# david-wb/tiny-diffusion

Measured on AMD Instinct MI355X. Metric: train images/s (q_sample+fwd+MSE+bwd+allreduce+Adam), MNIST 28x28 UNet fp32; 1000-step sample latency in `sample`, higher is better.
Workload: dtype f32; 1 GPU; diffusion.py unconditional MNIST 28x28 UNet, fp32, train step, batch 256/GPU (BASELINE.json configs[1]); global_batch=256, per_gpu_batch=256, parallelism=dp1

## Files before the change

### include/tdx.h

```cpp
#ifndef TDX_H
#define TDX_H

#include <stddef.h>
#include <stdint.h>

#ifdef __cplusplus
extern "C" {
#endif

#define TDX_VERSION 400

#define TDX_E_BADARG (-1)
#define TDX_E_SHAPE (-2)
#define TDX_E_WORKSPACE (-3)
#define TDX_E_STATE (-4)

typedef void* tdx_stream_t;

int tdx_version(void);
const char* tdx_error_string(int code);


int tdx_q_sample(const float* x0, const float* noise, const int64_t* t,
                 const float* sqrt_ac, const float* sqrt_1mac, float* x_t,
// ... 290 lines not shown
size_t tdx_vae_loss_scratch_bytes(void);
int tdx_vae_bce_logits_grad(const float* logits, const float* x, float* loss_out, float* d_logits, float* recon,
                            float gscale, int64_t n, void* scratch, tdx_stream_t stream);
int tdx_vae_kld_reparam_bwd(const float* mu, const float* logvar, const float* eps, const float* g_z, float* kld_out,
                            float* g_mu, float* g_logvar, float kld_weight, int64_t n, void* scratch,
                            tdx_stream_t stream);
int tdx_vae_reparameterize_philox(const float* mu, const float* logvar, float* z, float* eps_out, int64_t n,
                                  uint64_t seed, uint64_t offset, tdx_stream_t stream);
size_t tdx_vae_train_workspace_floats(int batch, int input_dim, int hidden_dim, int latent_dim);
int tdx_vae_loss_grads(const float* x, const void* const* params, void* const* grads, const float* eps, uint64_t seed,
                       uint64_t offset, float kld_weight, float gscale, float* out3, float* workspace, int batch,
                       int input_dim, int hidden_dim, int latent_dim, tdx_stream_t stream);

int tdx_layernorm_fwd(const float* x, const float* gamma, const float* beta, float* out,
                      float* mean, float* rstd, int M, int N, float eps, tdx_stream_t stream);
int tdx_layernorm_bwd(const float* gy, const float* x, const float* gamma, const float* mean,
                      const float* rstd, float* gx, float* dgamma, float* dbeta, int M, int N,
                      tdx_stream_t stream);
int tdx_act_fwd(const float* x, float* out, int64_t n, int kind, tdx_stream_t stream);
int tdx_act_bwd(const float* gy, const float* x, float* gx, int64_t n, int kind, tdx_stream_t stream);
int tdx_dropout(const float* x, float* out, int64_t n, int group, float p, uint64_t seed,
                uint64_t offset, tdx_stream_t stream);
int tdx_add(const float* a, const float* b, float* out, int64_t n, int64_t b_period, tdx_stream_t stream);
int tdx_embedding_fwd(const float* weight, const int64_t* idx, float* out, int M, int N,
                      tdx_stream_t stream);
int tdx_embedding_bwd(const float* g, const int64_t* idx, float* dweight, int M, int N, int num,
                      tdx_stream_t stream);

typedef struct tdx_transformer_shape {
  int batch, latent_dim, dim, num_heads, num_layers, num_classes;
  float dropout_p, ln_eps;
} tdx_transformer_shape;
size_t tdx_transformer_train_workspace_floats(const tdx_transformer_shape* shape);
int tdx_transformer_loss_grads(const tdx_transformer_shape* shape, const void* const* params, void* const* grads,
                               const float* z_t, const int64_t* t, const int64_t* y, const float* target,
                               const float* w_table, int train, uint64_t seed, uint64_t offset,
                               const uint64_t* rng_dev, float gscale, float* loss_out, float* eps_hat_out,
                               float* workspace, tdx_stream_t stream);

typedef struct tdx_unet tdx_unet;

int tdx_unet_create(tdx_unet** out, int max_batch, int num_classes);
enum { TDX_UNET_MNIST = 0, TDX_UNET_LAION = 1, TDX_UNET_LATENT_MLP = 2 };
int tdx_unet_create_ex(tdx_unet** out, int max_batch, int kind, int num_classes);
int tdx_unet_create_hw(tdx_unet** out, int max_batch, int kind, int num_classes, int hw);
int tdx_unet_create_full(tdx_unet** out, int max_batch, int kind, int num_classes, int hw, int time_dim);
typedef int (*tdx_allreduce_fn)(void* user, double* device_buffer, int n, tdx_stream_t stream);
int tdx_unet_set_bn_sync(tdx_unet* u, tdx_allreduce_fn fn, void* user, double* buffer);

int tdx_unet_set_streams(tdx_unet* u, int mode);

#define TDX_PREC_F32 0
#define TDX_PREC_BF16 1
int tdx_unet_set_precision(tdx_unet* u, int precision);
int tdx_unet_destroy(tdx_unet* u);
size_t tdx_unet_workspace_bytes(const tdx_unet* u, int batch, int mode);

int tdx_unet_forward(tdx_unet* u, const void* const* params, void* const* buffers,
                     const float* x, const int64_t* t, const void* cond, float* out,
                     void* workspace, size_t workspace_bytes, int batch, int mode,
                     tdx_stream_t stream);

int tdx_unet_backward_stages(void);
int tdx_unet_backward(tdx_unet* u, const void* const* params, void* const* grads,
                      const float* d_out, void* workspace, size_t workspace_bytes,
                      int batch, int stage_lo, int stage_hi, tdx_stream_t stream);
int tdx_unet_backward_join(tdx_unet* u, tdx_stream_t stream);
int tdx_unet_backward_mark(tdx_unet* u, int slot);
int tdx_unet_backward_wait_mark(tdx_unet* u, int slot, tdx_stream_t stream);
int tdx_unet_backward_sync_mark(tdx_unet* u, int slot);

int tdx_unet_request_input_grad(tdx_unet* u, float* g_x);

int tdx_timestep_embedding(const int64_t* t, float* out, int B, int dim, tdx_stream_t stream);
int tdx_timestep_embedding_f32(const float* t, float* out, int B, int dim, tdx_stream_t stream);

int tdx_time_mlp_fwd(const int64_t* t, const int64_t* y, const void* const* params, float* pre,
                     float* emb, float* t1, float* t2, float* t3, int batch, tdx_stream_t stream);
int tdx_time_mlp_bwd(const int64_t* t, const int64_t* y, const void* const* params,
                     void* const* grads, const float* pre, const float* emb, const float* g_t1,
                     const float* g_t2, const float* g_t3, float* scratch, int batch,
                     int num_classes, tdx_stream_t stream);

int tdx_unet_eval_step(tdx_unet* u, const void* const* params, void* const* buffers, float* x,
                       const void* cond, const float* z, const float* coef, int64_t* counter,
                       int32_t* t_idx, int64_t* t_vec, float* eps, int64_t n_elems,
                       void* workspace, size_t workspace_bytes, int batch, uint64_t philox_seed,
                       tdx_stream_t stream);

int tdx_unet_prepare_sampling(tdx_unet* u, const void* const* params, const void* cond, int batch, int T,
                              tdx_stream_t stream);

int tdx_unet_drop_sampling_tables(tdx_unet* u);

int tdx_unet_prepare_sampling_sched(tdx_unet* u, const void* const* params, const void* cond, int batch,
                                    const int64_t* tau, int S, tdx_stream_t stream);
int tdx_unet_eval_step_update(tdx_unet* u, const void* const* params, void* const* buffers, float* x,
                              const void* cond, const float* z, const float* coef, const int64_t* tau, int S,
                              int64_t* counter, int32_t* t_idx, int64_t* t_vec, float* eps, int64_t n_elems,
                              void* workspace, size_t workspace_bytes, int batch, uint64_t philox_seed, int form,
                              int guided, float w, float lo, float hi, float* hist, const float* known,
                              const float* mask, tdx_stream_t stream);
int tdx_unet_eval_step_update_dyn(tdx_unet* u, const void* const* params, void* const* buffers, float* x,
                                  const void* cond, const float* z, const float* coef, const int64_t* tau, int S,
                                  int64_t* counter, int32_t* t_idx, int64_t* t_vec, float* eps, int64_t n_elems,
                                  void* workspace, size_t workspace_bytes, int batch, uint64_t philox_seed, int form,
                                  int guided, float w, float lo, float hi, float* hist, const float* known,
                                  const float* mask, int rank, float frac, float* thr, tdx_stream_t stream);

int tdx_unet_tensor(const tdx_unet* u, int batch, const char* name, size_t* offset_floats,
                    size_t* numel);

int tdx_unet_pack(tdx_unet* u, const void* const* params, void* const* buffers,
                  tdx_stream_t stream);

int tdx_tune_set(const char* key, int value);
int tdx_tune_get(const char* key, int* value);
const char* tdx_tune_name(int index);

int tdx_diag_set_buffer(void* device_buffer, size_t bytes);
int tdx_diag_conv_occupancy(int tile);

int tdx_probe_mfma_f32(float* out, int iters, int blocks, tdx_stream_t stream);
int tdx_probe_stream_copy(const float* src, float* dst, int64_t n, tdx_stream_t stream);

#ifdef __cplusplus
}
#endif
#endif
```

### tiny_diffusion_amd/_lib.py

```python
from __future__ import annotations

import contextlib
import ctypes as C
import os

import torch

from . import _build

_c_float_p = C.c_void_p
_c_i64_p = C.c_void_p
_ptr = C.c_void_p


class TdxError(RuntimeError):
    pass


def _load():
    path = _build.LIB
    if not os.path.exists(path):
        if os.environ.get("TDX_NO_AUTOBUILD"):
            raise TdxError(
                f"{path} not found: build it with `python -m tiny_diffusion_amd._build` "
# ... 122 lines not shown
    "tdx_vae_decode": (C.c_int, [_ptr, _ptr, _ptr, _ptr, C.c_int, C.c_int, C.c_int, C.c_int, _ptr]),
    "tdx_vae_loss_scratch_bytes": (C.c_size_t, []),
    "tdx_vae_bce_logits_grad": (C.c_int, [_ptr] * 5 + [C.c_float, C.c_int64, _ptr, _ptr]),
    "tdx_vae_kld_reparam_bwd": (C.c_int, [_ptr] * 7 + [C.c_float, C.c_int64, _ptr, _ptr]),
    "tdx_vae_reparameterize_philox": (C.c_int, [_ptr] * 4 + [C.c_int64, C.c_uint64, C.c_uint64, _ptr]),
    "tdx_vae_train_workspace_floats": (C.c_size_t, [C.c_int] * 4),
    "tdx_vae_loss_grads": (C.c_int, [_ptr] * 4 + [C.c_uint64, C.c_uint64, C.c_float, C.c_float, _ptr, _ptr]
                           + [C.c_int] * 4 + [_ptr]),
    "tdx_layernorm_fwd": (C.c_int, [_ptr, _ptr, _ptr, _ptr, _ptr, _ptr, C.c_int, C.c_int, C.c_float, _ptr]),
    "tdx_layernorm_bwd": (C.c_int, [_ptr, _ptr, _ptr, _ptr, _ptr, _ptr, _ptr, _ptr, C.c_int, C.c_int, _ptr]),
    "tdx_act_fwd": (C.c_int, [_ptr, _ptr, C.c_int64, C.c_int, _ptr]),
    "tdx_act_bwd": (C.c_int, [_ptr, _ptr, _ptr, C.c_int64, C.c_int, _ptr]),
    "tdx_dropout": (C.c_int, [_ptr, _ptr, C.c_int64, C.c_int, C.c_float, C.c_uint64, C.c_uint64, _ptr]),
    "tdx_add": (C.c_int, [_ptr, _ptr, _ptr, C.c_int64, C.c_int64, _ptr]),
    "tdx_embedding_fwd": (C.c_int, [_ptr, _ptr, _ptr, C.c_int, C.c_int, _ptr]),
    "tdx_embedding_bwd": (C.c_int, [_ptr, _ptr, _ptr, C.c_int, C.c_int, C.c_int, _ptr]),
    "tdx_transformer_train_workspace_floats": (C.c_size_t, [_ptr]),
    "tdx_transformer_loss_grads": (C.c_int, [_ptr] * 8 + [C.c_int, C.c_uint64, C.c_uint64, _ptr, C.c_float] + [_ptr] * 4),
    "tdx_unet_create": (C.c_int, [C.POINTER(_ptr), C.c_int, C.c_int]),
    "tdx_unet_create_ex": (C.c_int, [C.POINTER(_ptr), C.c_int, C.c_int, C.c_int]),
    "tdx_unet_create_hw": (C.c_int, [C.POINTER(_ptr), C.c_int, C.c_int, C.c_int, C.c_int]),
    "tdx_unet_create_full": (C.c_int, [C.POINTER(_ptr), C.c_int, C.c_int, C.c_int, C.c_int, C.c_int]),
    "tdx_unet_set_bn_sync": (C.c_int, [_ptr, _ptr, _ptr, _ptr]),
    "tdx_unet_set_streams": (C.c_int, [_ptr, C.c_int]),
    "tdx_unet_set_precision": (C.c_int, [_ptr, C.c_int]),
    "tdx_pack_conv3x3_bf16": (C.c_int, [_ptr, _ptr, _ptr, C.c_int, C.c_int, _ptr]),
    "tdx_conv3x3_bf16_stat_tile_rows": (C.c_int, []),
    "tdx_conv3x3_fwd_bf16": (C.c_int, [_ptr, _ptr, _ptr, _ptr, C.c_int, C.c_int, C.c_int, C.c_int, C.c_int,
                                       C.c_int, _ptr, _ptr, _ptr, _ptr, _ptr, _ptr]),
    "tdx_conv3x3_wgrad_bf16": (C.c_int, [_ptr, _ptr, _ptr, C.c_int, C.c_int, C.c_int, C.c_int, C.c_int,
                                         C.c_int, _ptr, _ptr, _ptr]),
    "tdx_unet_destroy": (C.c_int, [_ptr]),
    "tdx_unet_workspace_bytes": (C.c_size_t, [_ptr, C.c_int, C.c_int]),
    "tdx_unet_forward": (C.c_int, [_ptr, _ptr, _ptr, _ptr, _ptr, _ptr, _ptr, _ptr, C.c_size_t, C.c_int,
                                   C.c_int, _ptr]),
    "tdx_unet_backward_stages": (C.c_int, []),
    "tdx_unet_backward": (C.c_int, [_ptr, _ptr, _ptr, _ptr, _ptr, C.c_size_t, C.c_int, C.c_int, C.c_int,
                                    _ptr]),
    "tdx_unet_backward_join": (C.c_int, [_ptr, _ptr]),
    "tdx_unet_backward_mark": (C.c_int, [_ptr, C.c_int]),
    "tdx_unet_backward_wait_mark": (C.c_int, [_ptr, C.c_int, _ptr]),
    "tdx_unet_backward_sync_mark": (C.c_int, [_ptr, C.c_int]),
    "tdx_unet_request_input_grad": (C.c_int, [_ptr, _ptr]),
    "tdx_unet_prepare_sampling": (C.c_int, [_ptr, _ptr, _ptr, C.c_int, C.c_int, _ptr]),
    "tdx_unet_drop_sampling_tables": (C.c_int, [_ptr]),
    "tdx_unet_prepare_sampling_sched": (C.c_int, [_ptr, _ptr, _ptr, C.c_int, _ptr, C.c_int, _ptr]),
    "tdx_initial_conv_input_grad": (C.c_int, [_ptr, _ptr, _ptr] + [C.c_int] * 5 + [_ptr]),
    "tdx_unet_eval_step": (C.c_int, [_ptr, _ptr, _ptr, _ptr, _ptr, _ptr, _ptr, _ptr, _ptr, _ptr, _ptr, C.c_int64,
                                     _ptr, C.c_size_t, C.c_int, C.c_uint64, _ptr]),
    "tdx_unet_eval_step_update": (C.c_int, [_ptr] * 8 + [C.c_int, _ptr, _ptr, _ptr, _ptr, C.c_int64, _ptr, C.c_size_t,
                                            C.c_int, C.c_uint64, C.c_int, C.c_int] + [C.c_float] * 3 + [_ptr] * 4),
    "tdx_p_sample_update": (C.c_int, [_ptr, _ptr, _ptr, C.c_int64, C.c_int, _ptr, _ptr, _ptr, _ptr, C.c_int, C.c_uint64,
                                      C.c_int, C.c_float, C.c_float, C.c_float, _ptr, _ptr, _ptr, _ptr, _ptr]),
    "tdx_x0_dyn_threshold": (C.c_int, [_ptr, _ptr, C.c_int, C.c_int, _ptr, _ptr, C.c_int, C.c_float, C.c_float, C.c_float,
                                       C.c_int, C.c_float, _ptr, _ptr]),
    "tdx_p_sample_update_dyn": (C.c_int, [_ptr, _ptr, _ptr, C.c_int64, C.c_int, _ptr, _ptr, _ptr, _ptr, C.c_int,
                                          C.c_uint64, C.c_int, C.c_float, C.c_float, C.c_float, _ptr, _ptr, _ptr, _ptr,
                                          _ptr, C.c_int, _ptr]),
    "tdx_unet_eval_step_update_dyn": (C.c_int, [_ptr] * 8 + [C.c_int, _ptr, _ptr, _ptr, _ptr, C.c_int64, _ptr, C.c_size_t,
                                                C.c_int, C.c_uint64, C.c_int, C.c_int] + [C.c_float] * 3 + [_ptr] * 3
                                      + [C.c_int, C.c_float, _ptr, _ptr]),
    "tdx_vlb_terms": (C.c_int, [_ptr] * 6 + [C.c_int, C.c_int] + [C.c_float] * 4 + [C.c_int, _ptr, C.c_int64, _ptr]),
    "tdx_p_sample_step_guided": (C.c_int, [_ptr, _ptr, _ptr, _ptr, _ptr, _ptr, C.c_int64, C.c_float, C.c_int,
                                           C.c_uint64, _ptr, _ptr]),
    "tdx_p_sample_step_x0": (C.c_int, [_ptr] * 7 + [C.c_int64, C.c_float, C.c_float, C.c_int, C.c_uint64, _ptr, _ptr]),
    "tdx_p_sample_step_x0_guided": (C.c_int, [_ptr] * 6 + [C.c_int64, C.c_float, C.c_float, C.c_float, C.c_int,
                                                           C.c_uint64, _ptr, _ptr]),
    "tdx_p_sample_step_ms": (C.c_int, [_ptr] * 6 + [C.c_int64, C.c_float, C.c_float, _ptr, _ptr]),
    "tdx_p_sample_step_ms_guided": (C.c_int, [_ptr] * 5 + [C.c_int64, C.c_float, C.c_float, C.c_float, _ptr, _ptr]),
    "tdx_p_sample_step_x0_masked": (C.c_int, [_ptr] * 9 + [C.c_int64, C.c_float, C.c_float, C.c_int, C.c_uint64, _ptr,
                                                           _ptr]),
    "tdx_p_sample_step_x0_guided_masked": (C.c_int, [_ptr] * 8 + [C.c_int64, C.c_float, C.c_float, C.c_float, C.c_int,
                                                                  C.c_uint64, _ptr, _ptr]),
    "tdx_p_sample_step_ms_masked": (C.c_int, [_ptr] * 8 + [C.c_int64, C.c_float, C.c_float, _ptr, _ptr]),
    "tdx_p_sample_step_ms_guided_masked": (C.c_int, [_ptr] * 7 + [C.c_int64, C.c_float, C.c_float, C.c_float, _ptr,
                                                                  _ptr]),
    "tdx_cond_drop_labels": (C.c_int, [_ptr, _ptr, C.c_int, C.c_float, C.c_uint64, C.c_uint64, _ptr]),
    "tdx_cond_drop_rows": (C.c_int, [_ptr, _ptr, C.c_int, C.c_int, C.c_float, C.c_uint64, C.c_uint64, _ptr]),
    "tdx_timestep_embedding": (C.c_int, [_ptr, _ptr, C.c_int, C.c_int, _ptr]),
    "tdx_timestep_embedding_f32": (C.c_int, [_ptr, _ptr, C.c_int, C.c_int, _ptr]),
    "tdx_time_mlp_fwd": (C.c_int, [_ptr, _ptr, _ptr, _ptr, _ptr, _ptr, _ptr, _ptr, C.c_int, _ptr]),
    "tdx_time_mlp_bwd": (C.c_int, [_ptr, _ptr, _ptr, _ptr, _ptr, _ptr, _ptr, _ptr, _ptr, _ptr, C.c_int, C.c_int,
                                   _ptr]),
    "tdx_conv3x3_dgrad": (C.c_int, [_ptr, _ptr, _ptr, C.c_int, C.c_int, C.c_int, C.c_int, C.c_int, _ptr]),
    "tdx_bn_apply_relu_fwd": (C.c_int, [_ptr, _ptr, C.c_int64, C.c_int, _ptr, _ptr, _ptr]),
    "tdx_unet_pack": (C.c_int, [_ptr, _ptr, _ptr, _ptr]),
    "tdx_unet_tensor": (C.c_int, [_ptr, C.c_int, C.c_char_p, C.POINTER(C.c_size_t), C.POINTER(C.c_size_t)]),
    "tdx_tune_set": (C.c_int, [C.c_char_p, C.c_int]),
    "tdx_tune_get": (C.c_int, [C.c_char_p, C.POINTER(C.c_int)]),
    "tdx_tune_name": (C.c_char_p, [C.c_int]),
    "tdx_diag_set_buffer": (C.c_int, [_ptr, C.c_size_t]),
    "tdx_probe_mfma_f32": (C.c_int, [_ptr, C.c_int, C.c_int, _ptr]),
    "tdx_probe_stream_copy": (C.c_int, [_ptr, _ptr, C.c_int64, _ptr]),
}

EXPORTS = tuple(_SIGS)
STEP_EPS, STEP_X0, STEP_MS = 0, 1, 2


def _bind():
    missing = []
    for name, (res, args) in _SIGS.items():
        try:
            fn = getattr(lib, name)
        except AttributeError:
            missing.append(name)
            continue
        fn.restype = res
        fn.argtypes = args
    if missing:
        raise TdxError(f"libtdx.so lacks symbols declared in include/tdx.h: {missing}")


_bind()


def _apply_env_tuning():
    spec = os.environ.get("TDX_TUNE", "")
    for item in filter(None, (x.strip() for x in spec.split(","))):
        key, _, val = item.partition("=")
        if lib.tdx_tune_set(key.encode(), int(val)) != 0:
            raise TdxError(f"unknown TDX_TUNE knob {key!r}")


_apply_env_tuning()


def check(code: int, what: str = "tdx"):
    if code != 0:
        msg = lib.tdx_error_string(code)
        raise TdxError(f"{what} failed: {msg.decode() if msg else code} ({code})")


def tune_get(key: str) -> int:
    value = C.c_int()
    if lib.tdx_tune_get(key.encode(), C.byref(value)) != 0:
        raise TdxError(f"unknown tuning knob {key!r}")
    return value.value


@contextlib.contextmanager
def tuned(**knobs):
    old = [(key, tune_get(key)) for key in knobs]
    try:
        for key, value in knobs.items():
            check(lib.tdx_tune_set(key.encode(), int(value)), f"tdx_tune_set({key})")
        yield
    finally:
        for key, value in reversed(old):
            check(lib.tdx_tune_set(key.encode(), value), f"tdx_tune_set({key})")


def ptr(t):
    return None if t is None else t.data_ptr()


def stream_ptr(device=None):
    return torch.cuda.current_stream(device).cuda_stream
```

### tiny_diffusion_amd/csrc/time_embed.hip

```cpp
#include "internal.h"

#define TD 256
#define TDL 768

__device__ static inline float silu_f(float x) { return x / (1.0f + expf(-x)); }
__device__ static inline float silu_grad_f(float x) {
  const float s = 1.0f / (1.0f + expf(-x));
  return s * (1.0f + x * (1.0f - s));
}

__device__ static inline void wave_dot4(const float* __restrict__ w0, int row_stride, const float4 v,
                                        int lane, float (&out)[4]) {
  float4 a[4];
#pragma unroll
  for (int k = 0; k < 4; ++k) a[k] = *reinterpret_cast<const float4*>(w0 + (size_t)k * row_stride + lane * 4);
#pragma unroll
  for (int k = 0; k < 4; ++k) out[k] = wave_sum(a[k].x * v.x + a[k].y * v.y + a[k].z * v.z + a[k].w * v.w);
}

__global__ void __launch_bounds__(256)
time_emb_kernel(const int64_t* __restrict__ t, const int64_t* __restrict__ y,
                const float* __restrict__ w1, const float* __restrict__ b1,
                const float* __restrict__ w2, const float* __restrict__ b2,
                const float* __restrict__ cls, float* __restrict__ pre_out,
// ... 162 lines not shown
    default: return TDX_E_SHAPE;
  }
  TDX_CHECK_LAUNCH();
  return 0;
}

static int time_embed_fwd_laion(const int64_t* t, const float* cond, const float* const* P, float* sin,
                                float* pre, float* emb, float* t1, float* t2, float* t3, int B, int td,
                                hipStream_t st) {
  sinusoid_kernel<int64_t><<<cdiv((int64_t)B * td, 256), 256, 0, st>>>(t, sin, B, td);
  TDX_CHECK_LAUNCH();
  int rc = linear_rows<false>(sin, P[TDX_P_TE0_W], P[TDX_P_TE0_B], nullptr, pre, B, td, td, st);
  if (rc) return rc;
  rc = linear_rows<true>(pre, P[TDX_P_TE2_W], P[TDX_P_TE2_B], cond, emb, B, td, td, st);
  if (rc) return rc;
  float* dst[3] = {t1, t2, t3};
  const int width[3] = {64, 128, 256};
  const int pw[3] = {TDX_P_TP1_W, TDX_P_TP2_W, TDX_P_TP3_W};
  for (int k = 0; k < 3; ++k) {
    rc = linear_rows<false>(emb, P[pw[k]], P[pw[k] + 1], nullptr, dst[k], B, width[k], td, st);
    if (rc) return rc;
  }
  return 0;
}

__global__ void time_l1_fwd_kernel(const int64_t* __restrict__ t, const float* __restrict__ w1,
                                   const float* __restrict__ b1, float* __restrict__ pre, float* __restrict__ tf,
                                   int B, int td) {
  const int i = blockIdx.x * blockDim.x + threadIdx.x;
  if (i >= B * td) return;
  const int n = i / td, j = i - n * td;
  const float v = (float)t[n];
  pre[i] = fmaf(w1[j], v, b1[j]);
  if (tf && j == 0) tf[n] = v;
}

__global__ void add_class_emb_kernel(float* __restrict__ emb, const float* __restrict__ cls,
                                     const int64_t* __restrict__ y, int B, int td) {
  const int i = blockIdx.x * blockDim.x + threadIdx.x;
  if (i >= B * td) return;
  const int n = i / td, j = i - n * td;
  const int64_t c = y[n];
  if (c >= 0) emb[i] += cls[(size_t)c * td + j];
}

static int time_embed_fwd_generic0(const int64_t* t, const int64_t* y, const float* const* P, float* tf,
                                   float* pre, float* emb, float* t1, float* t2, float* t3, int B, int td,
                                   hipStream_t st) {
  time_l1_fwd_kernel<<<cdiv((int64_t)B * td, 256), 256, 0, st>>>(t, P[TDX_P_TE0_W], P[TDX_P_TE0_B], pre, tf, B, td);
  TDX_CHECK_LAUNCH();
  int rc = linear_rows<true>(pre, P[TDX_P_TE2_W], P[TDX_P_TE2_B], nullptr, emb, B, td, td, st);
  if (rc) return rc;
  if (y) {
    add_class_emb_kernel<<<cdiv((int64_t)B * td, 256), 256, 0, st>>>(emb, P[TDX_P_CLASS_EMB], y, B, td);
    TDX_CHECK_LAUNCH();
  }
  float* dst[3] = {t1, t2, t3};
  const int width[3] = {128, 256, 512};
  const int pw[3] = {TDX_P_TP1_W, TDX_P_TP2_W, TDX_P_TP3_W};
  for (int k = 0; k < 3; ++k) {
    rc = linear_rows<false>(emb, P[pw[k]], P[pw[k] + 1], nullptr, dst[k], B, width[k], td, st);
    if (rc) return rc;
  }
  return 0;
}

int tdx_time_embed_fwd(int kind, const int64_t* t, const int64_t* y, const float* cond,
                       const float* const* P, float* sin, float* pre, float* emb, float* t1, float* t2,
                       float* t3, int B, hipStream_t st, int td) {
  if (td <= 0) td = kind == 1 ? TDL : TD;
  if (!td_ok(kind, td)) return TDX_E_SHAPE;
  if (kind == 1) return time_embed_fwd_laion(t, cond, P, sin, pre, emb, t1, t2, t3, B, td, st);
  if (td != TD) return time_embed_fwd_generic0(t, y, P, sin, pre, emb, t1, t2, t3, B, td, st);
  time_emb_kernel<<<dim3(B, 4), 256, 0, st>>>(t, y, P[TDX_P_TE0_W], P[TDX_P_TE0_B], P[TDX_P_TE2_W],
                                              P[TDX_P_TE2_B], P[TDX_P_CLASS_EMB], pre, emb, sin);
  TDX_CHECK_LAUNCH();
  time_proj_kernel<<<dim3(B, 14), 256, 0, st>>>(emb, P[TDX_P_TP1_W], P[TDX_P_TP1_B], P[TDX_P_TP2_W],
                                                P[TDX_P_TP2_B], P[TDX_P_TP3_W], P[TDX_P_TP3_B], t1,
                                                t2, t3);
  TDX_CHECK_LAUNCH();
  return 0;
}

__global__ void lin_wgrad_kernel(const float* __restrict__ g, const float* __restrict__ x,
                                 float* __restrict__ dw, float* __restrict__ db, int B, int O, int J,
                                 int ldg) {
  const int idx = blockIdx.x * blockDim.x + threadIdx.x;
  if (idx >= O * J) return;
  const int o = idx / J, j = idx - o * J;
  float s = 0.f, sb = 0.f;
#pragma unroll 8
  for (int n = 0; n < B; ++n) {
    const float gv = g[(size_t)n * ldg + o];
    s = fmaf(gv, x[(size_t)n * J + j], s);
    sb += gv;
  }
  dw[idx] = s;
  if (j == 0 && db) db[o] = sb;
}

__global__ void lin_dgrad_kernel(const float* __restrict__ g, const float* __restrict__ w,
                                 float* __restrict__ gx, int B, int O, int J, int accumulate, int ldg) {
  const int idx = blockIdx.x * blockDim.x + threadIdx.x;
  if (idx >= B * J) return;
  const int n = idx / J, j = idx - n * J;
  float s = accumulate ? gx[idx] : 0.f;
#pragma unroll 8
  for (int o = 0; o < O; ++o) s = fmaf(g[(size_t)n * ldg + o], w[(size_t)o * J + j], s);
  gx[idx] = s;
}

__global__ void __launch_bounds__(256)
time_l1_bwd_kernel(const float* __restrict__ g_h, const float* __restrict__ pre,
                   const float* tf, float* __restrict__ dw1, float* __restrict__ db1,
                   int B, int td) {
  __shared__ float red[2][8][32];
  const int cl = threadIdx.x & 31, sl = threadIdx.x >> 5;
  const int j = blockIdx.x * 32 + cl;
  const bool live = j < td;
  float sw = 0.f, sb = 0.f;
#pragma unroll 4
  for (int n = sl; n < B && live; n += 8) {
    const float gp = g_h[(size_t)n * td + j] * silu_grad_f(pre[(size_t)n * td + j]);
    sw = fmaf(gp, __hip_atomic_load(tf + n, __ATOMIC_RELAXED, __HIP_MEMORY_SCOPE_AGENT), sw);
    sb += gp;
  }
  red[0][sl][cl] = sw;
  red[1][sl][cl] = sb;
  __syncthreads();
  if (sl == 0) {
    sw = 0.f; sb = 0.f;
#pragma unroll
    for (int k = 0; k < 8; ++k) { sw += red[0][k][cl]; sb += red[1][k][cl]; }
    if (live) {
      dw1[j] = sw;
      db1[j] = sb;
    }
  }
}

unsigned* g_tdx_diag_buffer = nullptr;
size_t g_tdx_diag_bytes = 0;
extern "C" int tdx_diag_set_buffer(void* p, size_t bytes) {
  if (p && !bytes) return TDX_E_BADARG;
  g_tdx_diag_buffer = static_cast<unsigned*>(p);
  g_tdx_diag_bytes = p ? bytes : 0;
  return 0;
}

__global__ void silu_bwd_kernel(float* __restrict__ g, const float* __restrict__ pre, int n) {
  const int i = blockIdx.x * blockDim.x + threadIdx.x;
  if (i < n) g[i] *= silu_grad_f(pre[i]);
}

__global__ void silu_kernel(const float* __restrict__ pre, float* __restrict__ h, int n) {
  const int i = blockIdx.x * blockDim.x + threadIdx.x;
  if (i < n) h[i] = silu_f(pre[i]);
}

__global__ void class_emb_bwd_kernel(const float* __restrict__ g_emb, const int64_t* y,
                                     float* __restrict__ de, int B, int ncls, int td) {
  __shared__ int ys[256];
  const int idx = blockIdx.x * blockDim.x + threadIdx.x;
  const bool live = idx < ncls * td;
  const int c = live ? idx / td : 0, j = live ? idx - c * td : 0;
  const int* y32 = reinterpret_cast<const int*>(y);
  float s = 0.f;
  for (int n0 = 0; n0 < B; n0 += 256) {
    __syncthreads();
    if (n0 + (int)threadIdx.x < B)
      ys[threadIdx.x] = __hip_atomic_load(y32 + 2 * (n0 + threadIdx.x), __ATOMIC_RELAXED, __HIP_MEMORY_SCOPE_AGENT);
    __syncthreads();
    const int nn = min(256, B - n0);
    if (live)
      for (int n = 0; n < nn; ++n)
        if (ys[n] == c) s += g_emb[(size_t)(n0 + n) * td + j];
  }
  if (live) de[idx] = s;
}

static int time_embed_bwd_laion(const float* const* P, float* const* G, const float* sin, const float* pre,
                                const float* emb, const float* g_t1, const float* g_t2, const float* g_t3,
                                float* scratch, int B, int td, hipStream_t st, int parts) {
  float* g_emb = scratch;
  float* h = scratch + (size_t)B * td;
  float* g_h = scratch + (size_t)2 * B * td;
  const float* gk[3] = {g_t1, g_t2, g_t3};
  const int ok[3] = {64, 128, 256};
  const int pw[3] = {TDX_P_TP1_W, TDX_P_TP2_W, TDX_P_TP3_W};
  for (int k = 0; k < 3 && (parts & TDX_TIME_PROJ); ++k) {
    lin_wgrad_kernel<<<cdiv(ok[k] * td, 256), 256, 0, st>>>(gk[k], emb, G[pw[k]], G[pw[k] + 1], B, ok[k], td, ok[k]);
    TDX_CHECK_LAUNCH();
    lin_dgrad_kernel<<<cdiv(B * td, 256), 256, 0, st>>>(gk[k], P[pw[k]], g_emb, B, ok[k], td, k > 0, ok[k]);
    TDX_CHECK_LAUNCH();
  }
  if (!(parts & TDX_TIME_MID)) return 0;
  silu_kernel<<<cdiv(B * td, 256), 256, 0, st>>>(pre, h, B * td);
  TDX_CHECK_LAUNCH();
  lin_wgrad_kernel<<<cdiv(td * td, 256), 256, 0, st>>>(g_emb, h, G[TDX_P_TE2_W], G[TDX_P_TE2_B], B, td, td, td);
  TDX_CHECK_LAUNCH();
  lin_dgrad_kernel<<<cdiv(B * td, 256), 256, 0, st>>>(g_emb, P[TDX_P_TE2_W], g_h, B, td, td, 0, td);
  TDX_CHECK_LAUNCH();
  silu_bwd_kernel<<<cdiv(B * td, 256), 256, 0, st>>>(g_h, pre, B * td);
  TDX_CHECK_LAUNCH();
  lin_wgrad_kernel<<<cdiv(td * td, 256), 256, 0, st>>>(g_h, sin, G[TDX_P_TE0_W], G[TDX_P_TE0_B], B, td, td, td);
  TDX_CHECK_LAUNCH();
  return 0;
}

int tdx_time_embed_bwd_ex(const float* tf, const int64_t* y, const float* const* P, float* const* G,
                          const float* pre, const float* emb, const float* const* gk, const int* ldg,
                          const int* widths, float* scratch, int B, int ncls, hipStream_t st, int td, int parts) {
  if (td <= 0) td = TD;
  float* g_emb = scratch;
  float* h = scratch + (size_t)B * td;
  float* g_h = scratch + (size_t)2 * B * td;
  const int pw[3] = {TDX_P_TP1_W, TDX_P_TP2_W, TDX_P_TP3_W};
  for (int k = 0; k < 3 && (parts & TDX_TIME_PROJ); ++k) {
    lin_wgrad_kernel<<<cdiv(widths[k] * td, 256), 256, 0, st>>>(gk[k], emb, G[pw[k]], G[pw[k] + 1], B,
                                                                widths[k], td, ldg[k]);
    TDX_CHECK_LAUNCH();
    lin_dgrad_kernel<<<cdiv(B * td, 256), 256, 0, st>>>(gk[k], P[pw[k]], g_emb, B, widths[k], td, k > 0,
                                                        ldg[k]);
    TDX_CHECK_LAUNCH();
  }
  if (parts & TDX_TIME_MID) {
    if (ncls > 0 && y) {
      class_emb_bwd_kernel<<<cdiv(ncls * td, 256), 256, 0, st>>>(g_emb, y, G[TDX_P_CLASS_EMB], B, ncls, td);
      TDX_CHECK_LAUNCH();
    }
    silu_kernel<<<cdiv(B * td, 256), 256, 0, st>>>(pre, h, B * td);
    TDX_CHECK_LAUNCH();
    lin_wgrad_kernel<<<cdiv(td * td, 256), 256, 0, st>>>(g_emb, h, G[TDX_P_TE2_W], G[TDX_P_TE2_B], B, td, td, td);
    TDX_CHECK_LAUNCH();
    lin_dgrad_kernel<<<cdiv(B * td, 256), 256, 0, st>>>(g_emb, P[TDX_P_TE2_W], g_h, B, td, td, 0, td);
    TDX_CHECK_LAUNCH();
  }
  if (!(parts & TDX_TIME_L1)) return 0;
  time_l1_bwd_kernel<<<cdiv(td, 32), 256, 0, st>>>(g_h, pre, tf, G[TDX_P_TE0_W], G[TDX_P_TE0_B], B, td);
  TDX_CHECK_LAUNCH();
  return 0;
}

int tdx_time_embed_bwd(int kind, const int64_t* y, const float* const* P, float* const* G,
                       const float* sin, const float* pre, const float* emb, const float* g_t1,
                       const float* g_t2, const float* g_t3, float* scratch, int B, int ncls,
                       hipStream_t st, int td, int parts) {
  if (td <= 0) td = kind == 1 ? TDL : TD;
  if (!td_ok(kind, td)) return TDX_E_SHAPE;
  if (kind == 1)
    return time_embed_bwd_laion(P, G, sin, pre, emb, g_t1, g_t2, g_t3, scratch, B, td, st, parts);
  const float* gk[3] = {g_t1, g_t2, g_t3};
  const int widths[3] = {128, 256, 512};
  return tdx_time_embed_bwd_ex(sin, y, P, G, pre, emb, gk, widths, widths, scratch, B, ncls, st, td, parts);
}

int tdx_time_proj_bwd(int kind, int k, const float* const* P, float* const* G, const float* emb,
                      const float* g_tk, float* scratch, int B, hipStream_t st, int td) {
  if (td <= 0) td = kind == 1 ? TDL : TD;
  if (k < 0 || k > 2 || !td_ok(kind, td)) return TDX_E_SHAPE;
  const int w = (kind == 1 ? 64 : 128) << k;
  const int pw = k == 0 ? TDX_P_TP1_W : k == 1 ? TDX_P_TP2_W : TDX_P_TP3_W;
  lin_wgrad_kernel<<<cdiv(w * td, 256), 256, 0, st>>>(g_tk, emb, G[pw], G[pw + 1], B, w, td, w);
  TDX_CHECK_LAUNCH();
  lin_dgrad_kernel<<<cdiv(B * td, 256), 256, 0, st>>>(g_tk, P[pw], scratch, B, w, td, k > 0, w);
  TDX_CHECK_LAUNCH();
  return 0;
}

int tdx_time_embed_only(const int64_t* t, const int64_t* y, const float* const* P, float* pre, float* emb,
                        float* tf_out, int B, hipStream_t st) {
  time_emb_kernel<<<dim3(B, 4), 256, 0, st>>>(t, y, P[TDX_P_TE0_W], P[TDX_P_TE0_B], P[TDX_P_TE2_W],
                                              P[TDX_P_TE2_B], P[TDX_P_CLASS_EMB], pre, emb, tf_out);
  TDX_CHECK_LAUNCH();
  return 0;
}

__global__ void t_to_float_kernel(const int64_t* __restrict__ t, float* __restrict__ tf, int n) {
  const int i = blockIdx.x * blockDim.x + threadIdx.x;
  if (i < n) tf[i] = (float)t[i];
}

__global__ void iota_i64_kernel(int64_t* __restrict__ out, int n) {
  const int i = blockIdx.x * blockDim.x + threadIdx.x;
  if (i < n) out[i] = i;
}

size_t tdx_time_tables_index_floats(int T) { return (2 * (size_t)T + 3) & ~(size_t)3; }

int tdx_time_tables_build(int kind, const float* const* P, int T, int td, float* tab1, float* tab2, float* tab3,
                          float* scratch, hipStream_t st, const int64_t* tau) {
  if (td <= 0) td = kind == 1 ? TDL : TD;
  int64_t* tt = reinterpret_cast<int64_t*>(scratch);
  float* sin = scratch + tdx_time_tables_index_floats(T);
  float* pre = sin + (size_t)T * td;
  float* emb = pre + (size_t)T * td;
  if (tau) {
    TDX_HIP(hipMemcpyAsync(tt, tau, (size_t)T * sizeof(int64_t), hipMemcpyDeviceToDevice, st));
  } else {
    iota_i64_kernel<<<cdiv(T, 256), 256, 0, st>>>(tt, T);
    TDX_CHECK_LAUNCH();
  }
  return tdx_time_embed_fwd(kind, tt, nullptr, nullptr, P, sin, pre, emb, tab1, tab2, tab3, T, st, td);
}

__global__ void class_rows_kernel(const float* __restrict__ cls, const int64_t* __restrict__ y, float* __restrict__ out,
                                  int B, int td) {
  const int i = blockIdx.x * blockDim.x + threadIdx.x;
  if (i >= B * td) return;
  const int n = i / td, j = i - n * td;
  const int64_t c = y[n];
  out[i] = c >= 0 ? cls[(size_t)c * td + j] : 0.f;
}

int tdx_time_tables_cond(int kind, const float* const* P, const void* cond, int B, int td, float* tabc1, float* tabc2,
                         float* tabc3, float* scratch, hipStream_t st) {
  if (td <= 0) td = kind == 1 ? TDL : TD;
  const float* c = static_cast<const float*>(cond);
  if (kind == 0) {
    class_rows_kernel<<<cdiv((int64_t)B * td, 256), 256, 0, st>>>(P[TDX_P_CLASS_EMB], static_cast<const int64_t*>(cond),
                                                                  scratch, B, td);
    TDX_CHECK_LAUNCH();
    c = scratch;
  }
  float* dst[3] = {tabc1, tabc2, tabc3};
  const int pw[3] = {TDX_P_TP1_W, TDX_P_TP2_W, TDX_P_TP3_W};
  for (int k = 0; k < 3; ++k) {
    const int width = (kind == 1 ? 64 : 128) << k;
    const int rc = linear_rows<false>(c, P[pw[k]], nullptr, nullptr, dst[k], B, width, td, st);
    if (rc) return rc;
  }
  return 0;
}

__global__ void __launch_bounds__(256)
sample_head_kernel(const int64_t* __restrict__ counter, int32_t* __restrict__ t_idx, int64_t* __restrict__ t_vec,
                   int B, int T, int w1, int w2, int w3, const float* __restrict__ tab1,
                   const float* __restrict__ tab2, const float* __restrict__ tab3, const float* __restrict__ tc1,
                   const float* __restrict__ tc2, const float* __restrict__ tc3, float* __restrict__ o1,
                   float* __restrict__ o2, float* __restrict__ o3, int B0, float* __restrict__ o1b,
                   float* __restrict__ o2b, float* __restrict__ o3b, const int64_t* __restrict__ tau) {
  const int64_t t64 = *counter;
  const int t = (int)(t64 < 0 ? 0 : t64 >= T ? T - 1 : t64);
  const int wsum = w1 + w2 + w3;
  const int i = blockIdx.x * blockDim.x + threadIdx.x;
  if (i < B) t_vec[i] = tau ? tau[t] : t64;
  if (i == 0) *t_idx = (int32_t)t64;
  if (i >= B * wsum) return;
  const int b = i / wsum, j = i - b * wsum;
// ... 47 lines not shown
```

Measured before the change: 27520 images/s.

## Replace naive time-MLP linear wgrad/dgrad with shared-memory tiled kernels

Swaps the one-output-per-thread linear weight-gradient and input-gradient kernels in the time-embedding backward for 64x64 shared-memory tiled GEMM kernels. Each thread computes a 4x4 register tile, and the next K-chunk is prefetched into registers while the current one is consumed. This targets redundant global loads in the small dense layers of the time MLP backward. It also exposes the two kernels through the C API. The bias reduction is folded into the wgrad tile, and vectorized loads are chosen at run time from alignment checks.

```diff
diff --git a/include/tdx.h b/include/tdx.h
--- a/include/tdx.h
+++ b/include/tdx.h
@@ -396,6 +396,11 @@
                      const float* g_t2, const float* g_t3, float* scratch, int batch,
                      int num_classes, tdx_stream_t stream);
 
+int tdx_lin_wgrad(const float* g, const float* x, float* dw, float* db, int B, int O, int J, int ldg,
+                  tdx_stream_t stream);
+int tdx_lin_dgrad(const float* g, const float* w, float* gx, int B, int O, int J, int accumulate, int ldg,
+                  tdx_stream_t stream);
+
 int tdx_unet_eval_step(tdx_unet* u, const void* const* params, void* const* buffers, float* x,
                        const void* cond, const float* z, const float* coef, int64_t* counter,
                        int32_t* t_idx, int64_t* t_vec, float* eps, int64_t n_elems,
diff --git a/tiny_diffusion_amd/_lib.py b/tiny_diffusion_amd/_lib.py
--- a/tiny_diffusion_amd/_lib.py
+++ b/tiny_diffusion_amd/_lib.py
@@ -228,6 +228,8 @@
     "tdx_time_mlp_fwd": (C.c_int, [_ptr, _ptr, _ptr, _ptr, _ptr, _ptr, _ptr, _ptr, C.c_int, _ptr]),
     "tdx_time_mlp_bwd": (C.c_int, [_ptr, _ptr, _ptr, _ptr, _ptr, _ptr, _ptr, _ptr, _ptr, _ptr, C.c_int, C.c_int,
                                    _ptr]),
+    "tdx_lin_wgrad": (C.c_int, [_ptr, _ptr, _ptr, _ptr, C.c_int, C.c_int, C.c_int, C.c_int, _ptr]),
+    "tdx_lin_dgrad": (C.c_int, [_ptr, _ptr, _ptr, C.c_int, C.c_int, C.c_int, C.c_int, C.c_int, _ptr]),
     "tdx_conv3x3_dgrad": (C.c_int, [_ptr, _ptr, _ptr, C.c_int, C.c_int, C.c_int, C.c_int, C.c_int, _ptr]),
     "tdx_bn_apply_relu_fwd": (C.c_int, [_ptr, _ptr, C.c_int64, C.c_int, _ptr, _ptr, _ptr]),
     "tdx_unet_pack": (C.c_int, [_ptr, _ptr, _ptr, _ptr]),
diff --git a/tiny_diffusion_amd/csrc/time_embed.hip b/tiny_diffusion_amd/csrc/time_embed.hip
--- a/tiny_diffusion_amd/csrc/time_embed.hip
+++ b/tiny_diffusion_amd/csrc/time_embed.hip
@@ -268,32 +268,190 @@
   return 0;
 }
 
-__global__ void lin_wgrad_kernel(const float* __restrict__ g, const float* __restrict__ x,
-                                 float* __restrict__ dw, float* __restrict__ db, int B, int O, int J,
-                                 int ldg) {
-  const int idx = blockIdx.x * blockDim.x + threadIdx.x;
-  if (idx >= O * J) return;
-  const int o = idx / J, j = idx - o * J;
-  float s = 0.f, sb = 0.f;
-#pragma unroll 8
-  for (int n = 0; n < B; ++n) {
-    const float gv = g[(size_t)n * ldg + o];
-    s = fmaf(gv, x[(size_t)n * J + j], s);
-    sb += gv;
-  }
-  dw[idx] = s;
-  if (j == 0 && db) db[o] = sb;
-}
-
-__global__ void lin_dgrad_kernel(const float* __restrict__ g, const float* __restrict__ w,
-                                 float* __restrict__ gx, int B, int O, int J, int accumulate, int ldg) {
-  const int idx = blockIdx.x * blockDim.x + threadIdx.x;
-  if (idx >= B * J) return;
-  const int n = idx / J, j = idx - n * J;
-  float s = accumulate ? gx[idx] : 0.f;
-#pragma unroll 8
-  for (int o = 0; o < O; ++o) s = fmaf(g[(size_t)n * ldg + o], w[(size_t)o * J + j], s);
-  gx[idx] = s;
+#define LIN_T 64
+#define LIN_KC 32
+
+__device__ static inline float4 lin_ld4(const float* __restrict__ m, int row, int nrows, int col, int ncols, int ld,
+                                        bool vec) {
+  float4 v = make_float4(0.f, 0.f, 0.f, 0.f);
+  if (row >= nrows || col >= ncols) return v;
+  const float* p = m + (size_t)row * ld + col;
+  if (vec && col + 3 < ncols) return *reinterpret_cast<const float4*>(p);
+  v.x = p[0];
+  if (col + 1 < ncols) v.y = p[1];
+  if (col + 2 < ncols) v.z = p[2];
+  if (col + 3 < ncols) v.w = p[3];
+  return v;
+}
+
+__device__ static inline void lin_st4(float* __restrict__ m, int row, int nrows, int col, int ncols, int ld, bool vec,
+                                      const float (&v)[4]) {
+  if (row >= nrows || col >= ncols) return;
+  float* p = m + (size_t)row * ld + col;
+  if (vec && col + 3 < ncols) {
+    *reinterpret_cast<float4*>(p) = make_float4(v[0], v[1], v[2], v[3]);
+    return;
+  }
+  p[0] = v[0];
+  if (col + 1 < ncols) p[1] = v[1];
+  if (col + 2 < ncols) p[2] = v[2];
+  if (col + 3 < ncols) p[3] = v[3];
+}
+
+__global__ void __launch_bounds__(256)
+lin_wgrad_tiled_kernel(const float* __restrict__ g, const float* __restrict__ x, float* __restrict__ dw,
+                       float* __restrict__ db, int B, int O, int J, int ldg, int vec) {
+  __shared__ __attribute__((aligned(16))) float gs[LIN_KC][LIN_T];
+  __shared__ __attribute__((aligned(16))) float xs[LIN_KC][LIN_T];
+  const int tid = threadIdx.x, tj = tid & 15, to = tid >> 4;
+  const int o0 = blockIdx.x * LIN_T, j0 = blockIdx.y * LIN_T;
+  float acc[4][4], sb[4];
+#pragma unroll
+  for (int r = 0; r < 4; ++r) {
+    sb[r] = 0.f;
+#pragma unroll
+    for (int c = 0; c < 4; ++c) acc[r][c] = 0.f;
+  }
+  float4 pg[2], px[2];
+  auto fetch = [&](int n0) {
+#pragma unroll
+    for (int i = 0; i < 2; ++i) {
+      const int idx = tid + i * 256, k = idx >> 4, c = (idx & 15) * 4;
+      pg[i] = lin_ld4(g, n0 + k, B, o0 + c, O, ldg, vec & 1);
+      px[i] = lin_ld4(x, n0 + k, B, j0 + c, J, J, vec & 2);
+    }
+  };
+  auto step = [&](int k) {
+    const float4 a4 = *reinterpret_cast<const float4*>(&gs[k][to * 4]);
+    const float4 b4 = *reinterpret_cast<const float4*>(&xs[k][tj * 4]);
+    const float a[4] = {a4.x, a4.y, a4.z, a4.w}, b[4] = {b4.x, b4.y, b4.z, b4.w};
+#pragma unroll
+    for (int r = 0; r < 4; ++r) {
+#pragma unroll
+      for (int c = 0; c < 4; ++c) acc[r][c] = fmaf(a[r], b[c], acc[r][c]);
+      sb[r] += a[r];
+    }
+  };
+  fetch(0);
+  for (int n0 = 0; n0 < B; n0 += LIN_KC) {
+    __syncthreads();
+#pragma unroll
+    for (int i = 0; i < 2; ++i) {
+      const int idx = tid + i * 256, k = idx >> 4, c = (idx & 15) * 4;
+      *reinterpret_cast<float4*>(&gs[k][c]) = pg[i];
+      *reinterpret_cast<float4*>(&xs[k][c]) = px[i];
+    }
+    __syncthreads();
+    if (n0 + LIN_KC < B) fetch(n0 + LIN_KC);
+    const int kmax = min(LIN_KC, B - n0);
+    if (kmax == LIN_KC) {
+#pragma unroll
+      for (int k = 0; k < LIN_KC; ++k) step(k);
+    } else {
+      for (int k = 0; k < kmax; ++k) step(k);
+    }
+  }
+#pragma unroll
+  for (int r = 0; r < 4; ++r) lin_st4(dw, o0 + to * 4 + r, O, j0 + tj * 4, J, J, vec & 4, acc[r]);
+  if (db && blockIdx.y == 0 && tj == 0) {
+#pragma unroll
+    for (int r = 0; r < 4; ++r)
+      if (o0 + to * 4 + r < O) db[o0 + to * 4 + r] = sb[r];
+  }
+}
+
+__global__ void __launch_bounds__(256)
+lin_dgrad_tiled_kernel(const float* __restrict__ g, const float* __restrict__ w, float* __restrict__ gx, int B, int O,
+                       int J, int accumulate, int ldg, int vec) {
+  __shared__ __attribute__((aligned(16))) float gs[LIN_KC][LIN_T + 4];
+  __shared__ __attribute__((aligned(16))) float ws[LIN_KC][LIN_T];
+  const int tid = threadIdx.x, tj = tid & 15, tn = tid >> 4;
+  const int nb = blockIdx.x * LIN_T, j0 = blockIdx.y * LIN_T;
+  float acc[4][4];
+#pragma unroll
+  for (int r = 0; r < 4; ++r) {
+    const float4 v = accumulate ? lin_ld4(gx, nb + tn * 4 + r, B, j0 + tj * 4, J, J, vec & 4)
+                                : make_float4(0.f, 0.f, 0.f, 0.f);
+    acc[r][0] = v.x; acc[r][1] = v.y; acc[r][2] = v.z; acc[r][3] = v.w;
+  }
+  float4 pg[2], pw[2];
+  auto fetch = [&](int o0) {
+#pragma unroll
+    for (int i = 0; i < 2; ++i) {
+      const int idx = tid + i * 256;
+      pg[i] = lin_ld4(g, nb + (idx >> 3), B, o0 + (idx & 7) * 4, O, ldg, vec & 1);
+      pw[i] = lin_ld4(w, o0 + (idx >> 4), O, j0 + (idx & 15) * 4, J, J, vec & 2);
+    }
+  };
+  auto step = [&](int k) {
+    const float4 a4 = *reinterpret_cast<const float4*>(&gs[k][tn * 4]);
+    const float4 b4 = *reinterpret_cast<const float4*>(&ws[k][tj * 4]);
+    const float a[4] = {a4.x, a4.y, a4.z, a4.w}, b[4] = {b4.x, b4.y, b4.z, b4.w};
+#pragma unroll
+    for (int r = 0; r < 4; ++r)
+#pragma unroll
+      for (int c = 0; c < 4; ++c) acc[r][c] = fmaf(a[r], b[c], acc[r][c]);
+  };
+  fetch(0);
+  for (int o0 = 0; o0 < O; o0 += LIN_KC) {
+    __syncthreads();
+#pragma unroll
+    for (int i = 0; i < 2; ++i) {
+      const int idx = tid + i * 256, n = idx >> 3, k = (idx & 7) * 4;
+      gs[k][n] = pg[i].x; gs[k + 1][n] = pg[i].y; gs[k + 2][n] = pg[i].z; gs[k + 3][n] = pg[i].w;
+      *reinterpret_cast<float4*>(&ws[idx >> 4][(idx & 15) * 4]) = pw[i];
+    }
+    __syncthreads();
+    if (o0 + LIN_KC < O) fetch(o0 + LIN_KC);
+    const int kmax = min(LIN_KC, O - o0);
+    if (kmax == LIN_KC) {
+#pragma unroll
+      for (int k = 0; k < LIN_KC; ++k) step(k);
+    } else {
+      for (int k = 0; k < kmax; ++k) step(k);
+    }
+  }
+#pragma unroll
+  for (int r = 0; r < 4; ++r) lin_st4(gx, nb + tn * 4 + r, B, j0 + tj * 4, J, J, vec & 4, acc[r]);
+}
+
+#define RC(call)            \
+  do {                      \
+    int rc__ = (call);      \
+    if (rc__) return rc__;  \
+  } while (0)
+
+static inline bool lin_al16(const void* p) { return (reinterpret_cast<uintptr_t>(p) & 15) == 0; }
+
+static int lin_wgrad(const float* g, const float* x, float* dw, float* db, int B, int O, int J, int ldg,
+                     hipStream_t st) {
+  const int vec = (lin_al16(g) && ldg % 4 == 0 ? 1 : 0) | (lin_al16(x) && J % 4 == 0 ? 2 : 0) |
+                  (lin_al16(dw) && J % 4 == 0 ? 4 : 0);
+  lin_wgrad_tiled_kernel<<<dim3(cdiv(O, LIN_T), cdiv(J, LIN_T)), 256, 0, st>>>(g, x, dw, db, B, O, J, ldg, vec);
+  TDX_CHECK_LAUNCH();
+  return 0;
+}
+
+static int lin_dgrad(const float* g, const float* w, float* gx, int B, int O, int J, int accumulate, int ldg,
+                     hipStream_t st) {
+  const int vec = (lin_al16(g) && ldg % 4 == 0 ? 1 : 0) | (lin_al16(w) && J % 4 == 0 ? 2 : 0) |
+                  (lin_al16(gx) && J % 4 == 0 ? 4 : 0);
+  lin_dgrad_tiled_kernel<<<dim3(cdiv(B, LIN_T), cdiv(J, LIN_T)), 256, 0, st>>>(g, w, gx, B, O, J, accumulate, ldg,
+                                                                              vec);
+  TDX_CHECK_LAUNCH();
+  return 0;
+}
+
+extern "C" int tdx_lin_wgrad(const float* g, const float* x, float* dw, float* db, int B, int O, int J, int ldg,
+                             tdx_stream_t stream) {
+  if (!g || !x || !dw || B <= 0 || O <= 0 || J <= 0 || ldg < O) return TDX_E_BADARG;
+  return lin_wgrad(g, x, dw, db, B, O, J, ldg, to_stream(stream));
+}
+
+extern "C" int tdx_lin_dgrad(const float* g, const float* w, float* gx, int B, int O, int J, int accumulate, int ldg,
+                             tdx_stream_t stream) {
+  if (!g || !w || !gx || B <= 0 || O <= 0 || J <= 0 || ldg < O) return TDX_E_BADARG;
+  return lin_dgrad(g, w, gx, B, O, J, accumulate, ldg, to_stream(stream));
 }
 
 __global__ void __launch_bounds__(256)
@@ -375,22 +533,17 @@
   const int ok[3] = {64, 128, 256};
   const int pw[3] = {TDX_P_TP1_W, TDX_P_TP2_W, TDX_P_TP3_W};
   for (int k = 0; k < 3 && (parts & TDX_TIME_PROJ); ++k) {
-    lin_wgrad_kernel<<<cdiv(ok[k] * td, 256), 256, 0, st>>>(gk[k], emb, G[pw[k]], G[pw[k] + 1], B, ok[k], td, ok[k]);
-    TDX_CHECK_LAUNCH();
-    lin_dgrad_kernel<<<cdiv(B * td, 256), 256, 0, st>>>(gk[k], P[pw[k]], g_emb, B, ok[k], td, k > 0, ok[k]);
-    TDX_CHECK_LAUNCH();
+    RC(lin_wgrad(gk[k], emb, G[pw[k]], G[pw[k] + 1], B, ok[k], td, ok[k], st));
+    RC(lin_dgrad(gk[k], P[pw[k]], g_emb, B, ok[k], td, k > 0, ok[k], st));
   }
   if (!(parts & TDX_TIME_MID)) return 0;
   silu_kernel<<<cdiv(B * td, 256), 256, 0, st>>>(pre, h, B * td);
   TDX_CHECK_LAUNCH();
-  lin_wgrad_kernel<<<cdiv(td * td, 256), 256, 0, st>>>(g_emb, h, G[TDX_P_TE2_W], G[TDX_P_TE2_B], B, td, td, td);
-  TDX_CHECK_LAUNCH();
-  lin_dgrad_kernel<<<cdiv(B * td, 256), 256, 0, st>>>(g_emb, P[TDX_P_TE2_W], g_h, B, td, td, 0, td);
-  TDX_CHECK_LAUNCH();
+  RC(lin_wgrad(g_emb, h, G[TDX_P_TE2_W], G[TDX_P_TE2_B], B, td, td, td, st));
+  RC(lin_dgrad(g_emb, P[TDX_P_TE2_W], g_h, B, td, td, 0, td, st));
   silu_bwd_kernel<<<cdiv(B * td, 256), 256, 0, st>>>(g_h, pre, B * td);
   TDX_CHECK_LAUNCH();
-  lin_wgrad_kernel<<<cdiv(td * td, 256), 256, 0, st>>>(g_h, sin, G[TDX_P_TE0_W], G[TDX_P_TE0_B], B, td, td, td);
-  TDX_CHECK_LAUNCH();
+  RC(lin_wgrad(g_h, sin, G[TDX_P_TE0_W], G[TDX_P_TE0_B], B, td, td, td, st));
   return 0;
 }
 
@@ -403,12 +556,8 @@
   float* g_h = scratch + (size_t)2 * B * td;
   const int pw[3] = {TDX_P_TP1_W, TDX_P_TP2_W, TDX_P_TP3_W};
   for (int k = 0; k < 3 && (parts & TDX_TIME_PROJ); ++k) {
-    lin_wgrad_kernel<<<cdiv(widths[k] * td, 256), 256, 0, st>>>(gk[k], emb, G[pw[k]], G[pw[k] + 1], B,
-                                                                widths[k], td, ldg[k]);
-    TDX_CHECK_LAUNCH();
-    lin_dgrad_kernel<<<cdiv(B * td, 256), 256, 0, st>>>(gk[k], P[pw[k]], g_emb, B, widths[k], td, k > 0,
-                                                        ldg[k]);
-    TDX_CHECK_LAUNCH();
+    RC(lin_wgrad(gk[k], emb, G[pw[k]], G[pw[k] + 1], B, widths[k], td, ldg[k], st));
+    RC(lin_dgrad(gk[k], P[pw[k]], g_emb, B, widths[k], td, k > 0, ldg[k], st));
   }
   if (parts & TDX_TIME_MID) {
     if (ncls > 0 && y) {
@@ -417,10 +566,8 @@
     }
     silu_kernel<<<cdiv(B * td, 256), 256, 0, st>>>(pre, h, B * td);
     TDX_CHECK_LAUNCH();
-    lin_wgrad_kernel<<<cdiv(td * td, 256), 256, 0, st>>>(g_emb, h, G[TDX_P_TE2_W], G[TDX_P_TE2_B], B, td, td, td);
-    TDX_CHECK_LAUNCH();
-    lin_dgrad_kernel<<<cdiv(B * td, 256), 256, 0, st>>>(g_emb, P[TDX_P_TE2_W], g_h, B, td, td, 0, td);
-    TDX_CHECK_LAUNCH();
+    RC(lin_wgrad(g_emb, h, G[TDX_P_TE2_W], G[TDX_P_TE2_B], B, td, td, td, st));
+    RC(lin_dgrad(g_emb, P[TDX_P_TE2_W], g_h, B, td, td, 0, td, st));
   }
   if (!(parts & TDX_TIME_L1)) return 0;
   time_l1_bwd_kernel<<<cdiv(td, 32), 256, 0, st>>>(g_h, pre, tf, G[TDX_P_TE0_W], G[TDX_P_TE0_B], B, td);
@@ -447,10 +594,8 @@
   if (k < 0 || k > 2 || !td_ok(kind, td)) return TDX_E_SHAPE;
   const int w = (kind == 1 ? 64 : 128) << k;
   const int pw = k == 0 ? TDX_P_TP1_W : k == 1 ? TDX_P_TP2_W : TDX_P_TP3_W;
-  lin_wgrad_kernel<<<cdiv(w * td, 256), 256, 0, st>>>(g_tk, emb, G[pw], G[pw + 1], B, w, td, w);
-  TDX_CHECK_LAUNCH();
-  lin_dgrad_kernel<<<cdiv(B * td, 256), 256, 0, st>>>(g_tk, P[pw], scratch, B, w, td, k > 0, w);
-  TDX_CHECK_LAUNCH();
+  RC(lin_wgrad(g_tk, emb, G[pw], G[pw + 1], B, w, td, w, st));
+  RC(lin_dgrad(g_tk, P[pw], scratch, B, w, td, k > 0, w, st));
   return 0;
 }
 
```

After: 27580 images/s (median of 6 runs). About the same (+0.2%).
